# doublemul/ADER

Hardware: AMD Instinct MI355X
Metric: train sessions/sec at batch=512 seq=50 (higher is better)
Workload: dtype bf16x3 (2^-16/product, fp32 accumulate); 1 GPU; synthetic 1M-item catalog, seq_len=50, batch=512/GPU, dense regime (BASELINE.json configs[4]); items=1000000, batch_per_gpu=512, global_batch=512, seq_len=50, hidden=150, blocks=2, heads=1, optimizer=dense TF-Adam, exchange=none, parallelism=dp1, session_tiles=one session per workgroup, rccl_ranks=1

## Files before the change

ader_amd/csrc/seq_bwd.hip:

```cpp
#include "seq_common.h"

#define RED_FLOATS (10 * 2 * HP)


__device__ __forceinline__ void flush_ln_partials(float (&dg)[10], float (&db)[10], float* red_l, float* __restrict__ slab, int b, int H,
                                                  int tid) {
    const int lane = tid & 63, wave = tid >> 6, sub = lane & 15;
#pragma unroll
    for (int i = 0; i < 10; ++i) {
        dg[i] += __shfl_xor(dg[i], 16, 64); dg[i] += __shfl_xor(dg[i], 32, 64);
        db[i] += __shfl_xor(db[i], 16, 64); db[i] += __shfl_xor(db[i], 32, 64);
    }
    if (lane < 16) {
#pragma unroll
        for (int i = 0; i < 10; ++i) {
            red_l[(wave * 2 + 0) * HP + sub + 16 * i] = dg[i];
            red_l[(wave * 2 + 1) * HP + sub + 16 * i] = db[i];
        }
    }
    lds_barrier();
    if (tid < 2 * HP) {
        const int which = tid / HP, c = tid - which * HP;
        float s = 0.0f;
#pragma unroll
        for (int w = 0; w < 10; ++w) s += red_l[(w * 2 + which) * HP + c];
        if (c < H) slab[((size_t)b * 2 + which) * H + c] = s;
    }
}

template <bool STORE>
__device__ __forceinline__ void ln_bwd_rows(float* Xf, const Out& ox, const Out& omean, const Out& ostd, const float (&gam)[10],
                                            const Out& odx, int T, int H, bool pruned, int tv0, int wave, int lane, float (&dg)[10],
                                            float (&db)[10]) {
    const int sub = lane & 15, rsub = lane >> 4;
#pragma unroll 1
    for (int pass = 0; pass < 2; ++pass) {
        const int t = 40 * pass + 4 * wave + rsub;
        if (t >= TR) continue;
        const bool valid = t < T && (!pruned || t == T - 1);
        const uint32_t bo = (uint32_t)(t * H + sub) * 4u;
        if (t < tv0) {
#pragma unroll
            for (int i = 0; i < 10; ++i) {
                const int c = sub + 16 * i;
                Xf[t * XS + c] = 0.0f;
                if (STORE) bstore(odx, (c < H) ? bo + 64u * i : OOB, 0.0f);
            }
            continue;
        }
        float xv[10];
#pragma unroll
        for (int i = 0; i < 10; ++i) xv[i] = bload(ox, (sub + 16 * i < H) ? bo + 64u * i : OOB);
        const float mean = bload(omean, (uint32_t)t * 4u);
        float sd = bload(ostd, (uint32_t)t * 4u);
        if (!valid) sd = 1.0f;
        const float rsd = 1.0f / sd;
        float xh[10], dxh[10], s1 = 0.0f, s2 = 0.0f;
#pragma unroll
        for (int i = 0; i < 10; ++i) {
            const int c = sub + 16 * i;
            const float g = (valid && c < H) ? Xf[t * XS + c] : 0.0f;
            xh[i] = (valid && c < H) ? (xv[i] - mean) * rsd : 0.0f;
            dxh[i] = g * gam[i];
            s1 += dxh[i];
            s2 += dxh[i] * xh[i];
            dg[i] += g * xh[i];
            db[i] += g;
        }
        s1 = row16_sum(s1) / (float)H;
        s2 = row16_sum(s2) / (float)H;
#pragma unroll
        for (int i = 0; i < 10; ++i) {
            const int c = sub + 16 * i;
            const float o = (valid && c < H) ? (dxh[i] - s1 - xh[i] * s2) * rsd : 0.0f;
            Xf[t * XS + c] = o;
            if (STORE) bstore(odx, (c < H) ? bo + 64u * i : OOB, o);
        }
    }
}

__device__ __forceinline__ void stage_rows(const Out& src, bf16* R, int H, int wave, int lane) {
    const int sub = lane & 15, rsub = lane >> 4;
#pragma unroll 1
    for (int pass = 0; pass < 2; ++pass) {
        const int t = 40 * pass + 4 * wave + rsub;
        if (t < TR) {
            const uint32_t bo = (uint32_t)(t * H + sub) * 4u;
            float v[10];
#pragma unroll
            for (int i = 0; i < 10; ++i) v[i] = bload(src, (sub + 16 * i < H) ? bo + 64u * i : OOB);
            bf16* Tp = R + t * LDR + sub;
#pragma unroll
            for (int i = 0; i < 10; ++i) put_split(Tp, Tp + TR * LDR, 16 * i, v[i]);
        }
    }
}

__global__ __launch_bounds__(640) void k_seq_bwd_ffn(AderSeqBwdFfn a) {
    extern __shared__ __attribute__((aligned(16))) unsigned char smem_raw[];
    bf16* R0 = (bf16*)smem_raw;
    bf16* R1 = R0 + RSZ;
    float* Xf = (float*)(R1 + RSZ);
    float* red_l = (float*)((bf16*)Xf + RSZ);
    int* sq_l = (int*)(red_l + RED_FLOATS);
    const int tid = threadIdx.x, lane = tid & 63, wave = tid >> 6;
    const int nb = wave % 5, mh = wave / 5;
    const int b = blockIdx.x, T = a.T, H = a.H;
    const bool pruned = a.pruned != 0;
    const uint32_t H4 = (uint32_t)H * 4u;
    const uint32_t didx_row0 = (uint32_t)b * (uint32_t)T * (uint32_t)H;
    bf16x8 bh[10], bl[10];
    {
        const int r = lane & 31, hh = lane >> 5;
        load_bfrags((const bf16*)a.w2 + 2 * WSZ, nb, r, hh, bh, bl);
    }
    if (tid < TR) sq_l[tid] = (tid < T) ? a.seq[(size_t)b * T + tid] : 0;
    float gam[10];
    load10(a.ln2_g, H, lane & 15, gam);
    lds_barrier();
    int tv0;
    {
        const unsigned long long nz = __ballot(lane < T && sq_l[lane] != 0);
        tv0 = nz ? (int)__ffsll((long long)nz) - 1 : T;
    }
    const bool skipw = mh == 0 && tv0 >= 32;
    {
        const Out odx = make_out(a.dx2, b, T, H, pruned), odh = make_out(a.dh2, b, T, H, pruned);
        const SDrop d2 = sdrop_of(a.d_ffn2, didx_row0);
        const int sub = lane & 15, rsub = lane >> 4;
#pragma unroll
        for (int pass = 0; pass < 2; ++pass) {
            const int t = 40 * pass + 4 * wave + rsub;
            if (t < tv0) {
                const uint32_t bo = (uint32_t)(t * H + sub) * 4u;
                bf16* Tp = R0 + t * LDR + sub;
#pragma unroll
                for (int i = 0; i < 10; ++i) {
                    const int c = sub + 16 * i;
                    Xf[t * XS + c] = 0.0f;
                    Tp[16 * i] = (bf16)0.0f; Tp[TR * LDR + 16 * i] = (bf16)0.0f;
                    bstore(odh, (c < H) ? bo + 64u * i : OOB, 0.0f);
                }
            } else if (t < TR) {
                const uint32_t bo = (uint32_t)(t * H + sub) * 4u;
                float v[10];
#pragma unroll
                for (int i = 0; i < 10; ++i) v[i] = bload(odx, (sub + 16 * i < H) ? bo + 64u * i : OOB);
                const bool live = sq_l[t] != 0;
                bf16* Tp = R0 + t * LDR + sub;
#pragma unroll
                for (int i = 0; i < 10; ++i) {
                    const int c = sub + 16 * i;
                    const float g = live ? v[i] : 0.0f;
                    Xf[t * XS + c] = g;
                    const float dh = sdrop_apply1(d2, didx_row0 + d2.off + (uint32_t)(t * H + c), g);
                    put_split(Tp, Tp + TR * LDR, 16 * i, dh);
                    bstore(odh, (c < H) ? bo + 64u * i : OOB, dh);
                }
            }
        }
    }
    lds_barrier();
    {
        PHASE_IDS;
        const Out oh = make_out(a.h1d, b, T, H, pruned), oda = make_out(a.da, b, T, H, pruned);
        const int t0 = 32 * mh + 4 * hh;
        const uint32_t boff0 = (n < H) ? (uint32_t)(t0 * H + n) * 4u : OOB;
        float h1[16];
#pragma unroll
        for (int j = 0; j < 16; ++j) h1[j] = bload(oh, boff0 + ROWJ(j) * H4);
        f32x16 acc = tile_mma(R0, mh, r, hh, bh, bl, skipw);
        load_bfrags((const bf16*)a.w1 + 2 * WSZ, nb, r, hh, bh, bl);
        bf16* Th = R1 + t0 * LDR + n;
        const float sc1 = a.d_ffn1.scale;
        if (skipw) {
#pragma unroll
            for (int j = 0; j < 16; ++j) bstore(oda, boff0 + ROWJ(j) * H4, 0.0f);
        } else {
#pragma unroll
            for (int j = 0; j < 16; ++j) {
                const float v = (h1[j] != 0.0f) ? acc[j] * sc1 : 0.0f;
                put_split(Th, Th + TR * LDR, ROWJ(j) * LDR, v);
                bstore(oda, boff0 + ROWJ(j) * H4, v);
            }
        }
    }
    lds_barrier();
    {
        PHASE_IDS;
        f32x16 acc = tile_mma(R1, mh, r, hh, bh, bl, skipw);
        float* Xp = Xf + (32 * mh + 4 * hh) * XS + n;
        if (!skipw) {
#pragma unroll
            for (int j = 0; j < 16; ++j) Xp[ROWJ(j) * XS] += acc[j];
        }
    }
    lds_barrier();
    float dg[10], db[10];
#pragma unroll
    for (int i = 0; i < 10; ++i) { dg[i] = 0.0f; db[i] = 0.0f; }
    {
        const Out ox = make_out(a.x1, b, T, H, pruned), om = make_out(a.mean2, b, T, 1, pruned), os = make_out(a.std2, b, T, 1, pruned);
        const Out odx1 = make_out(a.dx1, b, T, H, pruned);
        ln_bwd_rows<true>(Xf, ox, om, os, gam, odx1, T, H, pruned, tv0, wave, lane, dg, db);
    }
    flush_ln_partials(dg, db, red_l, a.slab, b, H, tid);
}

__global__ __launch_bounds__(640) void k_seq_bwd_qkv(AderSeqBwdQkv a) {
    extern __shared__ __attribute__((aligned(16))) unsigned char smem_raw[];
    bf16* R0 = (bf16*)smem_raw;
    bf16* R1 = R0 + RSZ;
    float* Xf = (float*)(R1 + RSZ);
    float* red_l = (float*)((bf16*)Xf + RSZ);
    int* sq_l = (int*)(red_l + RED_FLOATS);
    const int tid = threadIdx.x, lane = tid & 63, wave = tid >> 6;
    const int nb = wave % 5, mh = wave / 5;
    const int b = blockIdx.x, T = a.T, H = a.H;
    const bool pruned = a.pruned != 0;
    const uint32_t H4 = (uint32_t)H * 4u;
    bf16x8 bh[10], bl[10];
    {
        const int r = lane & 31, hh = lane >> 5;
        load_bfrags((const bf16*)a.wq + 2 * WSZ, nb, r, hh, bh, bl);
    }
    if (tid < TR) sq_l[tid] = (a.emb_bwd && tid < T) ? a.seq[(size_t)b * T + tid] : 1;
    int tv0;
    {
        const unsigned long long nz = __ballot(lane < T && a.seq[(size_t)b * T + (lane < T ? lane : 0)] != 0);
        tv0 = nz ? (int)__ffsll((long long)nz) - 1 : T;
    }
    const bool skipw = mh == 0 && tv0 >= 32;
    float gam[10];
    load10(a.ln1_g, H, lane & 15, gam);
    {
        const Out oq = make_out(a.dQ, b, T, H, pruned);
        stage_rows(oq, R0, H, wave, lane);
        const Out ok = make_out(a.dK, b, T, H, false);
        stage_rows(ok, R1, H, wave, lane);
    }
    lds_barrier();
    {
        PHASE_IDS;
        const Out ox1 = make_out(a.dx1, b, T, H, pruned);
        const int t0 = 32 * mh + 4 * hh;
        const uint32_t boff0 = (n < H) ? (uint32_t)(t0 * H + n) * 4u : OOB;
        float res[16];
#pragma unroll
        for (int j = 0; j < 16; ++j) res[j] = bload(ox1, boff0 + ROWJ(j) * H4);
        f32x16 acc = tile_mma(R0, mh, r, hh, bh, bl, skipw);
        load_bfrags((const bf16*)a.wk + 2 * WSZ, nb, r, hh, bh, bl);
        float* Xp = Xf + t0 * XS + n;
        if (!skipw) {
#pragma unroll
            for (int j = 0; j < 16; ++j) Xp[ROWJ(j) * XS] = acc[j] + res[j];
        }
    }
    lds_barrier();
    float dg[10], db[10];
#pragma unroll
    for (int i = 0; i < 10; ++i) { dg[i] = 0.0f; db[i] = 0.0f; }
    {
        const Out ov = make_out(a.dV, b, T, H, false);
        stage_rows(ov, R0, H, wave, lane);
        Out ox = make_out(a.x, b, T, H, false);
        const Out om = make_out(a.mean1, b, T, 1, pruned), os = make_out(a.std1, b, T, 1, pruned);
        ln_bwd_rows<false>(Xf, ox, om, os, gam, ox, T, H, pruned, tv0, wave, lane, dg, db);
    }
    lds_barrier();
    {
        PHASE_IDS;
        f32x16 acc = tile_mma(R1, mh, r, hh, bh, bl, skipw);
        load_bfrags((const bf16*)a.wv + 2 * WSZ, nb, r, hh, bh, bl);
        if (!skipw) {
            const bf16* Ah = R0 + (32 * mh + r) * LDR + 8 * hh;
            const bf16* Al = Ah + TR * LDR;
#pragma unroll
            for (int ks = 0; ks < 10; ++ks) {
                const bf16x8 ah = *(const bf16x8*)(Ah + 16 * ks);
                const bf16x8 al = *(const bf16x8*)(Al + 16 * ks);
                acc = mfma_bf16(al, bh[ks], acc);
                acc = mfma_bf16(ah, bl[ks], acc);
                acc = mfma_bf16(ah, bh[ks], acc);
            }
        }
        const Out odx = make_out(a.dx, b, T, H, false);
        const SDrop d0 = sdrop_of(a.d_emb, (uint32_t)b * (uint32_t)T * (uint32_t)H);
        const int t0 = 32 * mh + 4 * hh;
        const uint32_t boff0 = (n < H) ? (uint32_t)(t0 * H + n) * 4u : OOB;
        const uint32_t didx0 = (uint32_t)b * (uint32_t)T * (uint32_t)H + d0.off + (uint32_t)(t0 * H + n);
        const float* Xp = Xf + t0 * XS + n;
        if (skipw) {
#pragma unroll
            for (int j = 0; j < 16; ++j) bstore(odx, boff0 + ROWJ(j) * H4, 0.0f);
        } else {
#pragma unroll
            for (int j = 0; j < 16; ++j) {
                float v = Xp[ROWJ(j) * XS] + acc[j];
                if (a.emb_bwd) {
                    v = sdrop_apply1(d0, didx0 + ROWJ(j) * (uint32_t)H, v);
                    v = (sq_l[t0 + ROWJ(j)] != 0) ? v : 0.0f;
                }
                bstore(odx, boff0 + ROWJ(j) * H4, v);
            }
        }
    }
    flush_ln_partials(dg, db, red_l, a.slab, b, H, tid);
}

static const size_t kSeqBwdLds = (size_t)3 * RSZ * sizeof(bf16) + (size_t)RED_FLOATS * sizeof(float) + TR * sizeof(int);

static int check_dims(int B, int T, int H) {
    if (B <= 0) return 1;
    if (T < 1 || T > TR || H < 2 || H > 150 || (H & 1)) return -2;
    return 0;
}

extern "C" {

int ader_seq_bwd_ffn(const AderSeqBwdFfn* desc, void* stream) {
    const AderSeqBwdFfn& a = *desc;
    const int rc = check_dims(a.B, a.T, a.H);
    if (rc) return rc < 0 ? rc : 0;
    static bool attr_set_dev[ADER_MAX_DEV] = {};
    bool& attr_set = attr_set_dev[ader_cur_dev()];
    if (!attr_set) {
        hipError_t e = hipFuncSetAttribute((const void*)k_seq_bwd_ffn, hipFuncAttributeMaxDynamicSharedMemorySize, (int)kSeqBwdLds);
        if (e != hipSuccess) return (int)e;
        attr_set = true;
    }
    hipLaunchKernelGGL(k_seq_bwd_ffn, dim3(a.B), dim3(640), kSeqBwdLds, (hipStream_t)stream, a);
    HIP_LAUNCH_CHECK();
    return 0;
}

int ader_seq_bwd_qkv(const AderSeqBwdQkv* desc, void* stream) {
    const AderSeqBwdQkv& a = *desc;
    const int rc = check_dims(a.B, a.T, a.H);
    if (rc) return rc < 0 ? rc : 0;
    static bool attr_set_dev[ADER_MAX_DEV] = {};
    bool& attr_set = attr_set_dev[ader_cur_dev()];
    if (!attr_set) {
        hipError_t e = hipFuncSetAttribute((const void*)k_seq_bwd_qkv, hipFuncAttributeMaxDynamicSharedMemorySize, (int)kSeqBwdLds);
        if (e != hipSuccess) return (int)e;
        attr_set = true;
    }
    hipLaunchKernelGGL(k_seq_bwd_qkv, dim3(a.B), dim3(640), kSeqBwdLds, (hipStream_t)stream, a);
    HIP_LAUNCH_CHECK();
    return 0;
}

}
```

ader_amd/csrc/seq_common.h:

```cpp
#pragma once
#include "common.h"
#include "../../include/ader_hip.h"
#include <stddef.h>

typedef __bf16 bf16;
typedef bf16 bf16x8 __attribute__((ext_vector_type(8)));
typedef bf16 bf16x4 __attribute__((ext_vector_type(4)));

#define HP 160
#define LDR 168
#define WSZ (HP * LDR)
#define TR 64
#define XS 164
#define RSZ (2 * TR * LDR)
#define LDP 72

static_assert(sizeof(AderDrop) == sizeof(DropArgs), "AderDrop must mirror DropArgs");
static_assert(TR * XS * sizeof(float) <= RSZ * sizeof(bf16), "Xf must fit in one tile pair");

__device__ __forceinline__ f32x16 mfma_bf16(bf16x8 a, bf16x8 b, f32x16 c) {
    return __builtin_amdgcn_mfma_f32_32x32x16_bf16(a, b, c, 0, 0, 0);
}
__device__ __forceinline__ int acc_row(int reg, int hh) { return (reg & 3) + 8 * (reg >> 2) + 4 * hh; }
__device__ __forceinline__ bf16x4 tr_read(const bf16* p) {
    return __builtin_amdgcn_ds_read_tr16_b64_v4bf16((bf16x4 __attribute__((address_space(3)))*)p);
}
__device__ __forceinline__ bf16x8 cat4(bf16x4 a, bf16x4 b) {
    bf16x8 o;
#pragma unroll
    for (int j = 0; j < 4; ++j) { o[j] = a[j]; o[4 + j] = b[j]; }
    return o;
}
__device__ __forceinline__ int opaque(int v) { asm volatile("" : "+v"(v)); return v; }
#define PHASE_IDS                                             \
    const int lane_p = opaque(lane);                          \
    const int r = lane_p & 31, hh = lane_p >> 5;              \
    const int n = 32 * nb + r;                                \
    (void)hh; (void)n
__device__ __forceinline__ void lds_barrier() { asm volatile("s_waitcnt lgkmcnt(0)\n\ts_barrier" ::: "memory"); }
template <class D> __device__ __forceinline__ DropArgs drop_of(const D& d) {
    DropArgs o; o.key = d.key; o.thr = d.thr; o.scale = d.scale; o.base = d.base; o.split = d.split; o.base2 = d.base2;
    return o;
}
struct SDrop { uint32_t key, thr, off; float scale; };
template <class D> __device__ __forceinline__ SDrop sdrop_of(const D& d, uint32_t first_idx) {
    SDrop o;
    o.key = d.key; o.thr = d.thr; o.scale = d.thr ? d.scale : 1.0f;
    o.off = (first_idx >= d.split) ? d.base2 : d.base;
    return o;
}
template <bool ON> __device__ __forceinline__ float sdrop_apply(const SDrop& d, uint32_t idx_off, float x) {
    if (!ON) return x;
    return ((lowbias32(idx_off ^ d.key) >> 8) >= d.thr) ? x * d.scale : 0.0f;
}
__device__ __forceinline__ float sdrop_apply1(const SDrop& d, uint32_t idx_off, float x) {
    return d.thr ? sdrop_apply<true>(d, idx_off, x) : x;
}
__device__ __forceinline__ void put_split(bf16* Th, bf16* Tl, int off, float v) {
    const bf16 h = (bf16)v;
    Th[off] = h;
    Tl[off] = (bf16)(v - (float)h);
}

__device__ __forceinline__ void load_bfrags(const bf16* __restrict__ W, int nb, int r, int hh, bf16x8 (&bh)[10], bf16x8 (&bl)[10]) {
    const bf16* p = W + ((size_t)nb * 10 * 64 + 32 * hh + r) * 8;
#pragma unroll
    for (int ks = 0; ks < 10; ++ks) {
        bh[ks] = *(const bf16x8*)(p + 512 * ks);
        bl[ks] = *(const bf16x8*)(p + WSZ + 512 * ks);
    }
}
__device__ __forceinline__ f32x16 tile_mma(const bf16* Th, int mh, int r, int hh, const bf16x8 (&bh)[10], const bf16x8 (&bl)[10],
                                           bool skip = false) {
    const bf16* Ah = Th + (32 * mh + r) * LDR + 8 * hh;
    const bf16* Al = Ah + TR * LDR;
    f32x16 acc;
#pragma unroll
    for (int j = 0; j < 16; ++j) acc[j] = 0.0f;
    if (skip) return acc;
#pragma unroll
    for (int ks = 0; ks < 10; ++ks) {
        const bf16x8 ah = *(const bf16x8*)(Ah + 16 * ks);
        const bf16x8 al = *(const bf16x8*)(Al + 16 * ks);
        acc = mfma_bf16(al, bh[ks], acc);
        acc = mfma_bf16(ah, bl[ks], acc);
        acc = mfma_bf16(ah, bh[ks], acc);
    }
    return acc;
}

__device__ __forceinline__ void ln_row(const float* xr, bool valid, int H, int lane, const float (&g)[3], const float (&be)[3],
                                       float (&x)[3], float (&y)[3], float& mean, float& sd, float& xsum, float& ysum) {
    float s = 0.0f;
#pragma unroll
    for (int i = 0; i < 3; ++i) {
        const int c = lane + 64 * i;
        x[i] = (valid && c < H) ? xr[c] : 0.0f;
        s += x[i];
    }
    s = wave_sum(s);
    mean = s / (float)H;
    float q = 0.0f;
#pragma unroll
    for (int i = 0; i < 3; ++i) {
        const int c = lane + 64 * i;
        const float dlt = (c < H) ? (x[i] - mean) : 0.0f;
        q += dlt * dlt;
    }
    q = wave_sum(q);
    sd = sqrtf(q / (float)H + LN_EPS);
    float ys = 0.0f;
#pragma unroll
    for (int i = 0; i < 3; ++i) {
        const int c = lane + 64 * i;
        y[i] = 0.0f;
        if (valid && c < H) {
            y[i] = g[i] * ((x[i] - mean) / sd) + be[i];
            ys += y[i];
        }
    }
    xsum = s;
    ysum = wave_sum(ys);
}
#define DPP_F(v_, ctrl_) __builtin_bit_cast(float, __builtin_amdgcn_update_dpp(0, __builtin_bit_cast(int, (v_)), (ctrl_), 0xf, 0xf, false))
__device__ __forceinline__ float row16_sum(float v) {
    v += DPP_F(v, 0xB1);
    v += DPP_F(v, 0x4E);
    v += DPP_F(v, 0x141);
    v += DPP_F(v, 0x140);
    return v;
}
__device__ __forceinline__ void load10(const float* __restrict__ p, int H, int sub, float (&o)[10]) {
#pragma unroll
    for (int i = 0; i < 10; ++i) {
        const int c = sub + 16 * i;
        o[i] = (c < H) ? p[c] : 0.0f;
    }
}
__device__ __forceinline__ void load3(const float* __restrict__ p, int H, int lane, float (&o)[3]) {
#pragma unroll
    for (int i = 0; i < 3; ++i) {
        const int c = lane + 64 * i;
        o[i] = (c < H) ? p[c] : 0.0f;
    }
}

typedef __amdgpu_buffer_rsrc_t rsrc_t;
#define OOB 0x80000000u
struct Out { rsrc_t r; uint32_t sub; };
__device__ __forceinline__ Out make_out(const void* base, int b, int T, int row_elems, bool pruned) {
    Out o;
    const size_t first = pruned ? (size_t)b * row_elems : (size_t)b * T * row_elems;
    o.r = __builtin_amdgcn_make_buffer_rsrc((void*)((const float*)base + first), 0, (pruned ? row_elems : T * row_elems) * 4, 0x00020000);
    o.sub = pruned ? (uint32_t)(T - 1) * row_elems * 4u : 0u;
    return o;
}
__device__ __forceinline__ void bstore(const Out& o, uint32_t boff, float v) {
    __builtin_amdgcn_raw_buffer_store_b32(__builtin_bit_cast(uint32_t, v), o.r, (int)(boff - o.sub), 0, 2);
}
__device__ __forceinline__ float bload(const Out& o, uint32_t boff) {
    return __builtin_bit_cast(float, __builtin_amdgcn_raw_buffer_load_b32(o.r, (int)(boff - o.sub), 0, 0));
}
#define ROWJ(j) (((j) & 3) + 8 * ((j) >> 2))
__device__ __forceinline__ int opaque_s(int v) { asm volatile("" : "+s"(v)); return v; }
#define PRUNE_IDS                                                                      \
    const int rT = opaque_s(T) - 1;                                                    \
    const int mhT = rT >> 5, hhT = ((rT & 31) >> 2) & 1;                               \
    const int jT = 4 * ((rT & 31) >> 3) + (rT & 3), rjT = (rT & 3) + 8 * ((rT & 31) >> 3); \
    const bool act = !pruned || mh == mhT;                                             \
    (void)hhT; (void)jT; (void)rjT
__device__ __forceinline__ float pick16(const f32x16& a, int j) {
    float v = a[0];
#pragma unroll
    for (int i = 1; i < 16; ++i) v = (j == i) ? a[i] : v;
    return v;
}
```

ader_amd/csrc/seqp_common.h:

```cpp
#pragma once
#include "seq_common.h"

typedef float f32x4v __attribute__((ext_vector_type(4)));
__device__ __forceinline__ f32x4v mfma16_bf16(bf16x8 a, bf16x8 b, f32x4v c) {
    return __builtin_amdgcn_mfma_f32_16x16x32_bf16(a, b, c, 0, 0, 0);
}

#define OOBH 0x40000000u

__device__ __forceinline__ Out make_rows(const void* base, size_t first_row, int nrows, int row_elems) {
    Out o;
    o.r = __builtin_amdgcn_make_buffer_rsrc((void*)((const float*)base + first_row * row_elems), 0, nrows * row_elems * 4, 0x00020000);
    o.sub = 0u;
    return o;
}
__device__ __forceinline__ uint32_t row_base(bool pruned, int t, uint32_t rb, const int* info_l) {
    if (!pruned) return (uint32_t)t * rb;
    const int inf = info_l[t];
    return (inf & 64) ? (uint32_t)(inf >> 16) * rb : OOBH;
}


__device__ __forceinline__ void load_bfrags16(const bf16* __restrict__ W, int w, int lane, bf16x8 (&bh)[10], bf16x8 (&bl)[10]) {
    const int c = lane & 15, g = lane >> 4;
    const bf16* p = W + ((size_t)(w >> 1) * 10 * 64 + 32 * (g & 1) + 16 * (w & 1) + c) * 8 + (g >> 1) * 512;
#pragma unroll
    for (int ks = 0; ks < 5; ++ks) {
        bh[ks] = *(const bf16x8*)(p + 1024 * ks);
        bl[ks] = *(const bf16x8*)(p + WSZ + 1024 * ks);
    }
}
__device__ __forceinline__ void tile_mma16(const bf16* Th, int c, int g, const bf16x8 (&bh)[10], const bf16x8 (&bl)[10], int nrb, f32x4v (&acc)[2]) {
#pragma unroll
    for (int rb = 0; rb < 2; ++rb) {
        acc[rb] = (f32x4v){0.0f, 0.0f, 0.0f, 0.0f};
        if (rb >= nrb) continue;
        const bf16* Ah = Th + (16 * rb + c) * LDR + 8 * g;
#pragma unroll
        for (int ks = 0; ks < 5; ++ks) {
            const bf16x8 ah = *(const bf16x8*)(Ah + 32 * ks);
            const bf16x8 al = *(const bf16x8*)(Ah + TR * LDR + 32 * ks);
            acc[rb] = mfma16_bf16(al, bh[ks], acc[rb]);
            acc[rb] = mfma16_bf16(ah, bl[ks], acc[rb]);
            acc[rb] = mfma16_bf16(ah, bh[ks], acc[rb]);
        }
    }
}
```

Measured before the change: 236,200 sessions/s.

## Switch backward FFN/QKV GEMMs to 16x16x32 MFMA column-per-wave tiling

Replaces the 32x32 MFMA tiling (wave split into row-half and column block) with a layout where each wave owns a 16-column strip and iterates over four 16-row blocks using 16x16x32 bf16 MFMA. Weight fragments shrink to five k-steps per wave, and row blocks below the first valid token are skipped at row-block granularity. Global loads and stores become 64-bit buffer ops covering four columns, and the pruned path computes only the single final row block. This is meant to cut register pressure and wasted MFMA work on padded rows, at the cost of more LDS activation reads per weight fragment.

```diff
diff --git a/ader_amd/csrc/seq_bwd.hip b/ader_amd/csrc/seq_bwd.hip
--- a/ader_amd/csrc/seq_bwd.hip
+++ b/ader_amd/csrc/seq_bwd.hip
@@ -104,16 +104,12 @@
     float* red_l = (float*)((bf16*)Xf + RSZ);
     int* sq_l = (int*)(red_l + RED_FLOATS);
     const int tid = threadIdx.x, lane = tid & 63, wave = tid >> 6;
-    const int nb = wave % 5, mh = wave / 5;
     const int b = blockIdx.x, T = a.T, H = a.H;
     const bool pruned = a.pruned != 0;
     const uint32_t H4 = (uint32_t)H * 4u;
     const uint32_t didx_row0 = (uint32_t)b * (uint32_t)T * (uint32_t)H;
-    bf16x8 bh[10], bl[10];
-    {
-        const int r = lane & 31, hh = lane >> 5;
-        load_bfrags((const bf16*)a.w2 + 2 * WSZ, nb, r, hh, bh, bl);
-    }
+    bf16x8 bh[5], bl[5];
+    load_bfrags16((const bf16*)a.w2 + 2 * WSZ, wave, lane, bh, bl);
     if (tid < TR) sq_l[tid] = (tid < T) ? a.seq[(size_t)b * T + tid] : 0;
     float gam[10];
     load10(a.ln2_g, H, lane & 15, gam);
@@ -123,7 +119,7 @@
         const unsigned long long nz = __ballot(lane < T && sq_l[lane] != 0);
         tv0 = nz ? (int)__ffsll((long long)nz) - 1 : T;
     }
-    const bool skipw = mh == 0 && tv0 >= 32;
+    const int rb0 = (tv0 >= 32) ? 2 : 0;
     {
         const Out odx = make_out(a.dx2, b, T, H, pruned), odh = make_out(a.dh2, b, T, H, pruned);
         const SDrop d2 = sdrop_of(a.d_ffn2, didx_row0);
@@ -161,38 +157,64 @@
         }
     }
     lds_barrier();
-    {
-        PHASE_IDS;
-        const Out oh = make_out(a.h1d, b, T, H, pruned), oda = make_out(a.da, b, T, H, pruned);
-        const int t0 = 32 * mh + 4 * hh;
-        const uint32_t boff0 = (n < H) ? (uint32_t)(t0 * H + n) * 4u : OOB;
-        float h1[16];
-#pragma unroll
-        for (int j = 0; j < 16; ++j) h1[j] = bload(oh, boff0 + ROWJ(j) * H4);
-        f32x16 acc = tile_mma(R0, mh, r, hh, bh, bl, skipw);
-        load_bfrags((const bf16*)a.w1 + 2 * WSZ, nb, r, hh, bh, bl);
-        bf16* Th = R1 + t0 * LDR + n;
+    if (!pruned) {
+        COL_IDS;
+        const Out oh = make_out(a.h1d, b, T, H, false), oda = make_out(a.da, b, T, H, false);
+        const Off4 f = off4((uint32_t)(c * H + n) * 4u, n, H);
+        f32x4 h1[4];
+#pragma unroll
+        for (int rb = 0; rb < 4; ++rb) h1[rb] = bload4(oh, f, (uint32_t)(16 * rb) * H4);
+        f32x4 acc[4];
+        zero4(acc);
+        tile_mma16t_from(R0, c, g, bh, bl, rb0, acc);
+        load_bfrags16((const bf16*)a.w1 + 2 * WSZ, wave, lane, bh, bl);
         const float sc1 = a.d_ffn1.scale;
-        if (skipw) {
-#pragma unroll
-            for (int j = 0; j < 16; ++j) bstore(oda, boff0 + ROWJ(j) * H4, 0.0f);
+#pragma unroll
+        for (int rb = 0; rb < 4; ++rb) {
+            f32x4 v = (f32x4){0.0f, 0.0f, 0.0f, 0.0f};
+            if (rb >= rb0) {
+#pragma unroll
+                for (int i = 0; i < 4; ++i) v[i] = (h1[rb][i] != 0.0f) ? acc[rb][i] * sc1 : 0.0f;
+                put_split4(R1, (16 * rb + c) * LDR + n, v);
+            }
+            bstore4(oda, f, (uint32_t)(16 * rb) * H4, v);
+        }
+    } else {
+        COL_IDS;
+        PRUNE_ROW;
+        const Out oh = make_out(a.h1d, b, T, H, true), oda = make_out(a.da, b, T, H, true);
+        const Off4 f = off4((uint32_t)(rT * H + n) * 4u, n, H);
+        const f32x4 h1 = bload4(oh, f, 0u);
+        f32x4 acc = (f32x4){0.0f, 0.0f, 0.0f, 0.0f};
+        if (pact) acc = tile_mma16t_rb(R0, rT >> 4, c, g, bh, bl);
+        load_bfrags16((const bf16*)a.w1 + 2 * WSZ, wave, lane, bh, bl);
+        const float sc1 = a.d_ffn1.scale;
+        if (c == (rT & 15)) {
+            f32x4 v = (f32x4){0.0f, 0.0f, 0.0f, 0.0f};
+            if (pact) {
+#pragma unroll
+                for (int i = 0; i < 4; ++i) v[i] = (h1[i] != 0.0f) ? acc[i] * sc1 : 0.0f;
+                put_split4(R1, rT * LDR + n, v);
+            }
+            bstore4(oda, f, 0u, v);
+        }
+    }
+    lds_barrier();
+    {
+        COL_IDS;
+        if (!pruned) {
+            f32x4 acc[4];
+            zero4(acc);
+            tile_mma16t_from(R1, c, g, bh, bl, rb0, acc);
+#pragma unroll
+            for (int rb = 0; rb < 4; ++rb)
+                if (rb >= rb0) *(f32x4*)(Xf + (16 * rb + c) * XS + n) += acc[rb];
         } else {
-#pragma unroll
-            for (int j = 0; j < 16; ++j) {
-                const float v = (h1[j] != 0.0f) ? acc[j] * sc1 : 0.0f;
-                put_split(Th, Th + TR * LDR, ROWJ(j) * LDR, v);
-                bstore(oda, boff0 + ROWJ(j) * H4, v);
-            }
-        }
-    }
-    lds_barrier();
-    {
-        PHASE_IDS;
-        f32x16 acc = tile_mma(R1, mh, r, hh, bh, bl, skipw);
-        float* Xp = Xf + (32 * mh + 4 * hh) * XS + n;
-        if (!skipw) {
-#pragma unroll
-            for (int j = 0; j < 16; ++j) Xp[ROWJ(j) * XS] += acc[j];
+            PRUNE_ROW;
+            if (pact) {
+                const f32x4 acc = tile_mma16t_rb(R1, rT >> 4, c, g, bh, bl);
+                if (c == (rT & 15)) *(f32x4*)(Xf + rT * XS + n) += acc;
+            }
         }
     }
     lds_barrier();
@@ -215,22 +237,18 @@
     float* red_l = (float*)((bf16*)Xf + RSZ);
     int* sq_l = (int*)(red_l + RED_FLOATS);
     const int tid = threadIdx.x, lane = tid & 63, wave = tid >> 6;
-    const int nb = wave % 5, mh = wave / 5;
     const int b = blockIdx.x, T = a.T, H = a.H;
     const bool pruned = a.pruned != 0;
     const uint32_t H4 = (uint32_t)H * 4u;
-    bf16x8 bh[10], bl[10];
-    {
-        const int r = lane & 31, hh = lane >> 5;
-        load_bfrags((const bf16*)a.wq + 2 * WSZ, nb, r, hh, bh, bl);
-    }
+    bf16x8 bh[5], bl[5];
+    load_bfrags16((const bf16*)a.wq + 2 * WSZ, wave, lane, bh, bl);
     if (tid < TR) sq_l[tid] = (a.emb_bwd && tid < T) ? a.seq[(size_t)b * T + tid] : 1;
     int tv0;
     {
         const unsigned long long nz = __ballot(lane < T && a.seq[(size_t)b * T + (lane < T ? lane : 0)] != 0);
         tv0 = nz ? (int)__ffsll((long long)nz) - 1 : T;
     }
-    const bool skipw = mh == 0 && tv0 >= 32;
+    const int rb0 = (tv0 >= 32) ? 2 : 0;
     float gam[10];
     load10(a.ln1_g, H, lane & 15, gam);
     {
@@ -240,21 +258,29 @@
         stage_rows(ok, R1, H, wave, lane);
     }
     lds_barrier();
-    {
-        PHASE_IDS;
-        const Out ox1 = make_out(a.dx1, b, T, H, pruned);
-        const int t0 = 32 * mh + 4 * hh;
-        const uint32_t boff0 = (n < H) ? (uint32_t)(t0 * H + n) * 4u : OOB;
-        float res[16];
-#pragma unroll
-        for (int j = 0; j < 16; ++j) res[j] = bload(ox1, boff0 + ROWJ(j) * H4);
-        f32x16 acc = tile_mma(R0, mh, r, hh, bh, bl, skipw);
-        load_bfrags((const bf16*)a.wk + 2 * WSZ, nb, r, hh, bh, bl);
-        float* Xp = Xf + t0 * XS + n;
-        if (!skipw) {
-#pragma unroll
-            for (int j = 0; j < 16; ++j) Xp[ROWJ(j) * XS] = acc[j] + res[j];
-        }
+    if (!pruned) {
+        COL_IDS;
+        const Out ox1 = make_out(a.dx1, b, T, H, false);
+        const Off4 f = off4((uint32_t)(c * H + n) * 4u, n, H);
+        f32x4 res[4];
+#pragma unroll
+        for (int rb = 0; rb < 4; ++rb) res[rb] = bload4(ox1, f, (uint32_t)(16 * rb) * H4);
+        f32x4 acc[4];
+        zero4(acc);
+        tile_mma16t_from(R0, c, g, bh, bl, rb0, acc);
+        load_bfrags16((const bf16*)a.wk + 2 * WSZ, wave, lane, bh, bl);
+#pragma unroll
+        for (int rb = 0; rb < 4; ++rb)
+            if (rb >= rb0) *(f32x4*)(Xf + (16 * rb + c) * XS + n) = acc[rb] + res[rb];
+    } else {
+        COL_IDS;
+        PRUNE_ROW;
+        const Out ox1 = make_out(a.dx1, b, T, H, true);
+        const f32x4 res = bload4(ox1, off4((uint32_t)(rT * H + n) * 4u, n, H), 0u);
+        f32x4 acc = (f32x4){0.0f, 0.0f, 0.0f, 0.0f};
+        if (pact) acc = tile_mma16t_rb(R0, rT >> 4, c, g, bh, bl);
+        load_bfrags16((const bf16*)a.wk + 2 * WSZ, wave, lane, bh, bl);
+        if (pact && c == (rT & 15)) *(f32x4*)(Xf + rT * XS + n) = acc + res;
     }
     lds_barrier();
     float dg[10], db[10];
@@ -269,40 +295,32 @@
     }
     lds_barrier();
     {
-        PHASE_IDS;
-        f32x16 acc = tile_mma(R1, mh, r, hh, bh, bl, skipw);
-        load_bfrags((const bf16*)a.wv + 2 * WSZ, nb, r, hh, bh, bl);
-        if (!skipw) {
-            const bf16* Ah = R0 + (32 * mh + r) * LDR + 8 * hh;
-            const bf16* Al = Ah + TR * LDR;
-#pragma unroll
-            for (int ks = 0; ks < 10; ++ks) {
-                const bf16x8 ah = *(const bf16x8*)(Ah + 16 * ks);
-                const bf16x8 al = *(const bf16x8*)(Al + 16 * ks);
-                acc = mfma_bf16(al, bh[ks], acc);
-                acc = mfma_bf16(ah, bl[ks], acc);
-                acc = mfma_bf16(ah, bh[ks], acc);
-            }
-        }
+        COL_IDS;
+        f32x4 acc[4];
+        zero4(acc);
+        tile_mma16t_from(R1, c, g, bh, bl, rb0, acc);
+        load_bfrags16((const bf16*)a.wv + 2 * WSZ, wave, lane, bh, bl);
+        tile_mma16t_from(R0, c, g, bh, bl, rb0, acc);
         const Out odx = make_out(a.dx, b, T, H, false);
         const SDrop d0 = sdrop_of(a.d_emb, (uint32_t)b * (uint32_t)T * (uint32_t)H);
-        const int t0 = 32 * mh + 4 * hh;
-        const uint32_t boff0 = (n < H) ? (uint32_t)(t0 * H + n) * 4u : OOB;
-        const uint32_t didx0 = (uint32_t)b * (uint32_t)T * (uint32_t)H + d0.off + (uint32_t)(t0 * H + n);
-        const float* Xp = Xf + t0 * XS + n;
-        if (skipw) {
-#pragma unroll
-            for (int j = 0; j < 16; ++j) bstore(odx, boff0 + ROWJ(j) * H4, 0.0f);
-        } else {
-#pragma unroll
-            for (int j = 0; j < 16; ++j) {
-                float v = Xp[ROWJ(j) * XS] + acc[j];
+        const Off4 f = off4((uint32_t)(c * H + n) * 4u, n, H);
+        const uint32_t didx0 = (uint32_t)b * (uint32_t)T * (uint32_t)H + d0.off + (uint32_t)(c * H + n);
+#pragma unroll
+        for (int rb = 0; rb < 4; ++rb) {
+            const int t = 16 * rb + c;
+            f32x4 v = (f32x4){0.0f, 0.0f, 0.0f, 0.0f};
+            if (rb >= rb0) {
+                v = *(const f32x4*)(Xf + t * XS + n) + acc[rb];
                 if (a.emb_bwd) {
-                    v = sdrop_apply1(d0, didx0 + ROWJ(j) * (uint32_t)H, v);
-                    v = (sq_l[t0 + ROWJ(j)] != 0) ? v : 0.0f;
+                    const bool live = sq_l[t] != 0;
+#pragma unroll
+                    for (int i = 0; i < 4; ++i) {
+                        const float u = sdrop_apply1(d0, didx0 + (uint32_t)(16 * rb) * (uint32_t)H + (uint32_t)i, v[i]);
+                        v[i] = live ? u : 0.0f;
+                    }
                 }
-                bstore(odx, boff0 + ROWJ(j) * H4, v);
-            }
+            }
+            bstore4(odx, f, (uint32_t)(16 * rb) * H4, v);
         }
     }
     flush_ln_partials(dg, db, red_l, a.slab, b, H, tid);
diff --git a/ader_amd/csrc/seq_common.h b/ader_amd/csrc/seq_common.h
--- a/ader_amd/csrc/seq_common.h
+++ b/ader_amd/csrc/seq_common.h
@@ -89,6 +89,68 @@
     return acc;
 }
 
+template <int N>
+__device__ __forceinline__ void load_bfrags16(const bf16* __restrict__ W, int w, int lane, bf16x8 (&bh)[N], bf16x8 (&bl)[N]) {
+    static_assert(N >= 5, "five k-steps of 32");
+    const int c = lane & 15, g = lane >> 4;
+    const bf16* p = W + ((size_t)(w >> 1) * 10 * 64 + 32 * (g & 1) + 16 * (w & 1) + c) * 8 + (g >> 1) * 512;
+#pragma unroll
+    for (int ks = 0; ks < 5; ++ks) {
+        bh[ks] = *(const bf16x8*)(p + 1024 * ks);
+        bl[ks] = *(const bf16x8*)(p + WSZ + 1024 * ks);
+    }
+}
+__device__ __forceinline__ f32x4 mfma16x32(bf16x8 a, bf16x8 b, f32x4 c) {
+    return __builtin_amdgcn_mfma_f32_16x16x32_bf16(a, b, c, 0, 0, 0);
+}
+template <int RB0>
+__device__ __forceinline__ void tile_mma16t(const bf16* Th, int c, int g, const bf16x8 (&wh)[5], const bf16x8 (&wl)[5], f32x4 (&acc)[4]) {
+    const bf16* Xh = Th + c * LDR + 8 * g;
+#pragma unroll
+    for (int ks = 0; ks < 5; ++ks) {
+#pragma unroll
+        for (int rb = RB0; rb < 4; ++rb) {
+            const bf16x8 xh = *(const bf16x8*)(Xh + 16 * rb * LDR + 32 * ks);
+            const bf16x8 xl = *(const bf16x8*)(Xh + 16 * rb * LDR + TR * LDR + 32 * ks);
+            acc[rb] = mfma16x32(wh[ks], xl, acc[rb]);
+            acc[rb] = mfma16x32(wl[ks], xh, acc[rb]);
+            acc[rb] = mfma16x32(wh[ks], xh, acc[rb]);
+        }
+    }
+}
+__device__ __forceinline__ void tile_mma16t_from(const bf16* Th, int c, int g, const bf16x8 (&wh)[5], const bf16x8 (&wl)[5], int rb0,
+                                                 f32x4 (&acc)[4]) {
+    if (rb0) tile_mma16t<2>(Th, c, g, wh, wl, acc);
+    else tile_mma16t<0>(Th, c, g, wh, wl, acc);
+}
+__device__ __forceinline__ void zero4(f32x4 (&acc)[4]) {
+#pragma unroll
+    for (int rb = 0; rb < 4; ++rb) acc[rb] = (f32x4){0.0f, 0.0f, 0.0f, 0.0f};
+}
+__device__ __forceinline__ f32x4 tile_mma16t_rb(const bf16* Th, int rb, int c, int g, const bf16x8 (&wh)[5], const bf16x8 (&wl)[5]) {
+    const bf16* Xh = Th + (16 * rb + c) * LDR + 8 * g;
+    f32x4 acc = (f32x4){0.0f, 0.0f, 0.0f, 0.0f};
+#pragma unroll
+    for (int ks = 0; ks < 5; ++ks) {
+        const bf16x8 xh = *(const bf16x8*)(Xh + 32 * ks);
+        const bf16x8 xl = *(const bf16x8*)(Xh + TR * LDR + 32 * ks);
+        acc = mfma16x32(wh[ks], xl, acc);
+        acc = mfma16x32(wl[ks], xh, acc);
+        acc = mfma16x32(wh[ks], xh, acc);
+    }
+    return acc;
+}
+__device__ __forceinline__ void put_split4(bf16* Th, int off, f32x4 v) {
+    bf16x4 h, l;
+#pragma unroll
+    for (int i = 0; i < 4; ++i) {
+        h[i] = (bf16)v[i];
+        l[i] = (bf16)(v[i] - (float)h[i]);
+    }
+    *(bf16x4*)(Th + off) = h;
+    *(bf16x4*)(Th + TR * LDR + off) = l;
+}
+
 __device__ __forceinline__ void ln_row(const float* xr, bool valid, int H, int lane, const float (&g)[3], const float (&be)[3],
                                        float (&x)[3], float (&y)[3], float& mean, float& sd, float& xsum, float& ysum) {
     float s = 0.0f;
@@ -161,6 +223,25 @@
 __device__ __forceinline__ float bload(const Out& o, uint32_t boff) {
     return __builtin_bit_cast(float, __builtin_amdgcn_raw_buffer_load_b32(o.r, (int)(boff - o.sub), 0, 0));
 }
+struct Off4 { uint32_t lo, hi; };
+__device__ __forceinline__ Off4 off4(uint32_t boff, int n, int H) {
+    Off4 o;
+    o.lo = (n < H) ? boff : OOB;
+    o.hi = (n + 2 < H) ? boff + 8u : OOB;
+    return o;
+}
+typedef uint32_t u32x2 __attribute__((ext_vector_type(2)));
+typedef uint32_t u32x4 __attribute__((ext_vector_type(4)));
+__device__ __forceinline__ void bstore4(const Out& o, Off4 f, uint32_t add, f32x4 v) {
+    const u32x4 u = __builtin_bit_cast(u32x4, v);
+    __builtin_amdgcn_raw_buffer_store_b64(__builtin_shufflevector(u, u, 0, 1), o.r, (int)(f.lo + add - o.sub), 0, 2);
+    __builtin_amdgcn_raw_buffer_store_b64(__builtin_shufflevector(u, u, 2, 3), o.r, (int)(f.hi + add - o.sub), 0, 2);
+}
+__device__ __forceinline__ f32x4 bload4(const Out& o, Off4 f, uint32_t add) {
+    const u32x2 a = __builtin_amdgcn_raw_buffer_load_b64(o.r, (int)(f.lo + add - o.sub), 0, 0);
+    const u32x2 c = __builtin_amdgcn_raw_buffer_load_b64(o.r, (int)(f.hi + add - o.sub), 0, 0);
+    return __builtin_bit_cast(f32x4, __builtin_shufflevector(a, c, 0, 1, 2, 3));
+}
 #define ROWJ(j) (((j) & 3) + 8 * ((j) >> 2))
 __device__ __forceinline__ int opaque_s(int v) { asm volatile("" : "+s"(v)); return v; }
 #define PRUNE_IDS                                                                      \
@@ -169,6 +250,14 @@
     const int jT = 4 * ((rT & 31) >> 3) + (rT & 3), rjT = (rT & 3) + 8 * ((rT & 31) >> 3); \
     const bool act = !pruned || mh == mhT;                                             \
     (void)hhT; (void)jT; (void)rjT
+#define COL_IDS                                               \
+    const int lane_c = opaque(lane);                          \
+    const int c = lane_c & 15, g = lane_c >> 4;               \
+    const int n = 16 * wave + 4 * g
+#define PRUNE_ROW                                             \
+    const int rT = opaque_s(T) - 1;                           \
+    const bool pact = rT >= 16 * rb0;                         \
+    (void)pact
 __device__ __forceinline__ float pick16(const f32x16& a, int j) {
     float v = a[0];
 #pragma unroll
diff --git a/ader_amd/csrc/seqp_common.h b/ader_amd/csrc/seqp_common.h
--- a/ader_amd/csrc/seqp_common.h
+++ b/ader_amd/csrc/seqp_common.h
@@ -21,15 +21,6 @@
 }
 
 
-__device__ __forceinline__ void load_bfrags16(const bf16* __restrict__ W, int w, int lane, bf16x8 (&bh)[10], bf16x8 (&bl)[10]) {
-    const int c = lane & 15, g = lane >> 4;
-    const bf16* p = W + ((size_t)(w >> 1) * 10 * 64 + 32 * (g & 1) + 16 * (w & 1) + c) * 8 + (g >> 1) * 512;
-#pragma unroll
-    for (int ks = 0; ks < 5; ++ks) {
-        bh[ks] = *(const bf16x8*)(p + 1024 * ks);
-        bl[ks] = *(const bf16x8*)(p + WSZ + 1024 * ks);
-    }
-}
 __device__ __forceinline__ void tile_mma16(const bf16* Th, int c, int g, const bf16x8 (&bh)[10], const bf16x8 (&bl)[10], int nrb, f32x4v (&acc)[2]) {
 #pragma unroll
     for (int rb = 0; rb < 2; ++rb) {
```

Result: no change. 235,900 sessions/s, median of 3 (-0.1%).
